# rossumur/espflix

Hardware: AMD Instinct MI355X
Metric: MPEG-1 352x192 frames/s (higher is better)
Workload: dtype u8/int32; 1 GPU; 1024 streams/GPU x GOP(12) I+11P, 352x192 MPEG-1 ES resident in HBM, ids rank*1024.. per rank (BASELINE configs[2]; at 8 GPUs = configs[4], stream k on rank floor(k*8/8192)); streams_per_gpu=1024, streams_total=1024, es_bytes_per_gpu=46457181, parallelism=stream-partition x1, coefficients_per_gpu=44531885, ring_depth=2

## Files before the change

### espflix_amd/csrc/efx_api.hip

```cpp
#include <hip/hip_runtime.h>

#include <algorithm>
#include <memory>
#include <mutex>
#include <thread>

#include <cstdio>
#include <cstdlib>
#include <cstring>
#include <string>
#include <vector>

#include "efx.h"
#include "efx_internal.h"
#include "enc_core.h"
#include "parse_tm.h"
#include "sbc_enc_core.h"

namespace efx {
struct DemuxChunk;
__global__ void k_demux_scan(const uint8_t*, const uint64_t*, const uint32_t*, const uint32_t*, DemuxChunk*);
__global__ void k_demux_offsets(const uint32_t*, const uint32_t*, DemuxChunk*, uint8_t*, const uint64_t*, uint32_t*, uint32_t*);
__global__ void k_demux(const uint8_t*, const uint64_t*, const uint32_t*, const uint32_t*, const DemuxChunk*, uint8_t*, PesEntry*);
__global__ void k_demux_fused(const uint8_t*, const uint64_t*, const uint32_t*, const uint32_t*, DemuxChunk*, uint8_t*, PesEntry*, uint32_t*, uint32_t*,
                              uint32_t*);
__global__ void k_demux_audio_scan(const uint8_t*, const uint64_t*, const uint32_t*, const uint32_t*, DemuxChunk*);
__global__ void k_demux_audio_offsets(const uint32_t*, const uint32_t*, DemuxChunk*, uint32_t*);
__global__ void k_demux_audio(const uint8_t*, const uint64_t*, const uint32_t*, const uint32_t*, const DemuxChunk*, uint8_t*, const uint64_t*);
__global__ void k_ts_sequences(const uint8_t*, const uint64_t*, const uint32_t*, const uint32_t*, PesEntry*, IdxInfo*);
__global__ void k_idx_bins(const PesEntry*, const uint32_t*, const IdxInfo*, uint32_t, uint32_t*, size_t);
__global__ void k_index(const uint8_t*, const uint64_t*, int, PicInfo*, SliceTmp*, uint32_t*, uint32_t*, uint32_t*,
                        const uint32_t*, const PesEntry*, const uint32_t*, const uint32_t*, int64_t*, int64_t*, int, int, int);
__global__ void k_advance(StreamState*, const uint32_t*, int64_t*, const int64_t*, int, int, int, int32_t*);
__global__ void k_slice_scan(const PicInfo*, const uint32_t*, int, int, const uint32_t*, uint32_t*, DecodeCounters*);
__global__ void k_slice_emit(const PicInfo*, const SliceTmp*, const uint32_t*, const uint64_t*, const uint32_t*, int, int,
                             const uint32_t*, SliceDesc*, uint32_t*);
__global__ void k_parse(const uint8_t*, const SliceDesc*, DecodeCounters*, const TmTables*, MbRec*, TmU4*, uint32_t*, uint32_t*,
                        int, int);
__global__ void k_recon(const MbRec*, const uint32_t*, const uint32_t*, const uint32_t*, uint8_t*, int, int, int, const int32_t*, int, int);
__global__ void k_recon_all(const MbRec*, const uint32_t*, const uint32_t*, const uint32_t*, uint8_t*, int, int, int, const int32_t*, int, int,
                            int, uint32_t*, uint32_t*, int);

__global__ void k_frame_hash(const uint8_t*, int, uint64_t*);
__global__ void k_fill(uint32_t*, uint32_t, size_t);
__global__ void k_composite(const uint8_t*, const VideoTables*, const VideoLineTemplates*, FieldArgs, uint16_t*);
__global__ void k_pdm(const int16_t*, int, int, int32_t*, uint16_t*);
template <int FMT, int CHROMA>
__global__ void k_export(const uint8_t*, int, ExportArgs);
__global__ void k_enc_begin(EncArgs);
__global__ void k_enc_rows(EncArgs);
__global__ void k_enc_pack(EncArgs);
__global__ void k_sbc(const uint8_t*, size_t, int, int, SbcState*, const SbcTables*, int16_t*, size_t, uint32_t*, uint32_t*, int);
__global__ void k_sbc_frames(const uint8_t*, size_t, int, int, SbcFrameInfo*, uint32_t*, uint32_t*, SbcQueues*);
__global__ void k_sbc_plan(const SbcFrameInfo*, int, int, const SbcState*, SbcFramePlan*, uint32_t*, SbcQueues*, uint32_t*, int, int, uint32_t*,
                           uint32_t*, SbcExtraItem*, uint8_t*);
__global__ void k_sbc_par_stereo(const uint8_t*, size_t, int, int, const SbcState*, SbcState*, const SbcTables*, const SbcFrameInfo*, int16_t*,
                                 size_t, uint32_t*, int, SbcQueues*, const uint32_t*, int, const SbcExtraItem*, int);
__global__ void k_sbc_par_mono(const uint8_t*, size_t, int, int, const SbcState*, SbcState*, const SbcTables*, const SbcFrameInfo*, int16_t*,
                               size_t, uint32_t*, int, SbcQueues*, const uint32_t*, int, const SbcExtraItem*, int);
__global__ void k_sbc_gen(const uint8_t*, size_t, int, int, const SbcState*, SbcState*, const SbcTables*, const SbcFrameInfo*,
                          const SbcFramePlan*, int16_t*, size_t, int, SbcQueues*, const uint32_t*, int, const uint8_t*, int);
__global__ void k_sbc_finish(const uint8_t*, size_t, int, int, SbcState*, const SbcState*, const SbcTables*, int16_t*, size_t, uint32_t*,
                             uint32_t*, int, uint32_t*);
__global__ void k_sbc_enc(SbcEncArgs);
__global__ void k_sbc_enc_state(SbcEncArgs);
__global__ void k_mux(MuxArgs);
}

using namespace efx;

#ifndef EFX_SBC_WG_PER_CU
#define EFX_SBC_WG_PER_CU 4
#endif

#ifndef EFX_PARSE_STREAMS
#define EFX_PARSE_STREAMS 2
#endif
#ifndef EFX_SLOTS
#define EFX_SLOTS 3
#endif
constexpr int kParseStreams = EFX_PARSE_STREAMS;
constexpr int kMaxGroups = 16;
static_assert(kMaxGroups <= kExportMaxGroups, "k_export takes every reconstruction group of a call");
#ifndef EFX_RECON_MERGE
#define EFX_RECON_MERGE 1
#endif
constexpr int kReconMerge = EFX_RECON_MERGE;
#ifndef EFX_GROUP_STREAMS
#define EFX_GROUP_STREAMS 1024
#endif
constexpr int kGroupStreams = EFX_GROUP_STREAMS;
constexpr int kTimingRing = 64;
constexpr int kSlots = EFX_SLOTS;
constexpr int kUploads = 3;
constexpr size_t kReconSyncWords(size_t streams) { return (64 + streams) * 32; }

struct efx_ctx {
    efx_config cfg{};
    hipStream_t stream = nullptr;
    bool own_stream = false;
    bool pooled_streams = false;
    unsigned stream_serial = 0;
    std::string err;

    size_t es_cap = 0;
    bool decoded = false, results_valid = false;

    ParseTables* d_tables = nullptr;
    TmTables* d_tm_tables = nullptr;
    uint8_t* d_frames = nullptr;
    StreamState* d_state = nullptr;

    struct Upload {
        uint8_t* d_es = nullptr;
        uint64_t* d_stream_off = nullptr;
        uint32_t* d_stream_perm = nullptr;
        uint32_t* d_ts_len = nullptr;
        uint32_t* d_pkt_base = nullptr;
        uint32_t* d_es_len = nullptr;
        uint32_t* d_pes_count = nullptr;
        PesEntry* d_pes = nullptr;
        uint8_t* h_es = nullptr;
        uint8_t* h_meta = nullptr;
        std::vector<uint64_t> stream_off;
        std::vector<uint32_t> es_len;
        int n_streams = 0;
        int sort_groups = 1;
        size_t es_used = 0, ts_bytes = 0;
        bool ts_input = false, valid = false;
        hipEvent_t uploaded = nullptr;
        hipEvent_t last_read[kParseStreams] = {};
        hipEvent_t ev_demux[2] = {nullptr, nullptr};
        bool demux_timed = false;
    } up[kUploads];
    int cur_up = -1;
    struct Arena {
        uint8_t* base;
        size_t bytes;
        bool owned;
    };
    std::vector<Arena> arenas;
    hipStream_t copy_stream = nullptr;
    uint8_t* d_ts = nullptr;
    DemuxChunk* d_demux_chunks = nullptr;
    size_t pes_cap = 0;
    IdxInfo* d_idx_info = nullptr;
    uint64_t* d_ts_off = nullptr;
    uint32_t* d_idx_len = nullptr;
    uint32_t* d_idx_base = nullptr;
    PesEntry* d_idx_seq = nullptr;
    bool ts_ready = false;

    struct Slot {
        uint32_t* d_pic_count = nullptr;
        uint32_t* d_status = nullptr;
        DecodeCounters* d_counters = nullptr;
        MbRec* d_mbrecs = nullptr;
        TmU4* d_raw = nullptr;
        uint32_t* d_coefs = nullptr;
        PicInfo* d_pics = nullptr;
        SliceTmp* d_slices_tmp = nullptr;
        uint32_t* d_qtab = nullptr;
        uint32_t* d_slice_base = nullptr;
        SliceDesc* d_descs = nullptr;
        int64_t* d_pts = nullptr;
        int32_t* d_call_pos = nullptr;
        uint32_t* d_recon_sync = nullptr;
        hipEvent_t parse_done[kReconMerge] = {}, recon_done = nullptr, wrap_cleared = nullptr;
        int epoch = 0;
        int upload = 0;
    } slot[kSlots];
    struct TimingEvents {
        hipEvent_t ev[5] = {nullptr, nullptr, nullptr, nullptr, nullptr};
    };
    std::vector<TimingEvents> timing_ring;
    uint64_t timed_calls = 0;
    struct Group {
        int slot, first, count;
        int half0, halves;
    };
    Group groups[kMaxGroups];
    int n_groups = 0;
    hipEvent_t last_recon_done = nullptr;
    uint64_t recon_groups_unsynced = 0;
    int last_upload = 0;
    int last_n_streams = 0;
    bool last_ts_input = false;
    uint64_t subcalls = 0;
    uint64_t parse_calls = 0;
    uint8_t timing_groups[kTimingRing] = {};
    uint16_t timing_launches[kTimingRing] = {};
    uint16_t timing_leaders[kTimingRing] = {};
    hipStream_t parse_streams[kParseStreams] = {};
    VideoTables* d_video[2] = {nullptr, nullptr};
    VideoLineTemplates* d_video_lines[2] = {nullptr, nullptr};
    SbcTables* d_sbc_tables = nullptr;
    sbcenc::Tables* d_sbc_enc_tables = nullptr;
    uint32_t* d_mux_before = nullptr;
    size_t mux_before_cap = 0;
    int parse_wg_cap = 0;
    int opt_groups = 0;
    int opt_parse_cap = 0;
    int opt_recon_mode = 0;
    int opt_recon_waves = 0;
    int opt_recon_items = 16;
    int n_cus = 256;
    uint32_t* d_sbc_flags = nullptr;
    SbcState* d_sbc_next = nullptr;
    size_t sbc_flags_cap = 0;
    SbcFrameInfo* d_sbc_info = nullptr;
    SbcFramePlan* d_sbc_plan = nullptr;
    SbcExtraItem* d_sbc_extra = nullptr;
    uint8_t* d_sbc_cover = nullptr;
    size_t sbc_info_cap = 0;
    size_t sbc_gran_cap = 0;
    int opt_sbc_serial = 0;
    int opt_demux_fused = 0;
    bool sbc_flags_clean = false;
    uint64_t* d_hash = nullptr;

    EncState* d_enc_state = nullptr;
    uint8_t* d_enc_pics = nullptr;
    uint8_t* d_enc_slices = nullptr;
    uint32_t* d_enc_slice_len = nullptr;
    enc::Tables* d_enc_tables = nullptr;
    std::unique_ptr<enc::Tables> h_enc_tables;
    uint32_t* h_enc_full = nullptr;
    uint32_t* d_enc_full = nullptr;
    bool enc_ready = false;
    bool enc_started = false;
    uint32_t enc_generation = 0;
    int enc_n_streams = 0, enc_format = 0, enc_gop = 0;

    int n_streams = 0;
    std::vector<int64_t> h_pts;
    std::vector<uint32_t> h_pic_count, h_status;
    std::vector<int32_t> h_call_pos;
    DecodeCounters h_counters{};

    bool timing = false;
};

namespace {

struct StreamSet {
    hipStream_t recon = nullptr, parse[kParseStreams] = {}, copy = nullptr;
    unsigned serial = 0;
// ... 200 lines not shown
    if (ctx->cfg.max_stream_bytes == 0)
        ctx->cfg.max_stream_bytes = (size_t)16384 * cfg->max_pictures * cfg->max_streams;
    auto bail = [&](int code) {
        efx_destroy(ctx);
        return code;
    };
    if (hipSetDevice(cfg->device) != hipSuccess)
        return bail(EFX_ERR_NO_DEVICE);
    StreamSet pooled;
    if (!cfg->hip_stream && take_stream_set(cfg->device, &pooled)) {
        ctx->stream = pooled.recon;
        ctx->own_stream = true;
        for (int i = 0; i < kParseStreams; i++)
            ctx->parse_streams[i] = pooled.parse[i];
        ctx->copy_stream = pooled.copy;
        ctx->pooled_streams = true;
        ctx->stream_serial = pooled.serial;
    } else if (cfg->hip_stream)
        ctx->stream = (hipStream_t)cfg->hip_stream;
    else {
        if (hipStreamCreateWithFlags(&ctx->stream, hipStreamNonBlocking) != hipSuccess)
            return bail(EFX_ERR_DEVICE);
        ctx->own_stream = true;
        ctx->pooled_streams = true;
        std::lock_guard<std::mutex> lk(g_pool_guard);
        ctx->stream_serial = ++g_set_serial;
    }
    if (!ctx->parse_streams[0]) {
        int lo = 0, hi = 0;
        if (hipDeviceGetStreamPriorityRange(&lo, &hi) != hipSuccess)
            return bail(EFX_ERR_DEVICE);
        for (auto& ps : ctx->parse_streams)
            if (hipStreamCreateWithPriority(&ps, hipStreamNonBlocking, hi) != hipSuccess)
                return bail(EFX_ERR_DEVICE);
        if (hipStreamCreateWithFlags(&ctx->copy_stream, hipStreamNonBlocking) != hipSuccess)
            return bail(EFX_ERR_DEVICE);
        std::vector<hipStream_t> order = {ctx->stream};
        for (auto ps : ctx->parse_streams)
            order.push_back(ps);
        order.push_back(ctx->copy_stream);
        for (hipStream_t st : order) {
            hipLaunchKernelGGL(k_fill, dim3(1), dim3(64), 0, st, (uint32_t*)nullptr, 0u, (size_t)0);
            if (hipStreamSynchronize(st) != hipSuccess)
                return bail(EFX_ERR_DEVICE);
        }
    }
    const size_t n = (size_t)cfg->max_streams, P = (size_t)cfg->max_pictures, D = (size_t)ctx->cfg.ring_depth;
    ctx->es_cap = ctx->cfg.max_stream_bytes + n * (kEsTailBytes + 32) + kEsGuardBytes;
    ctx->es_cap = (ctx->es_cap + 255) & ~(size_t)255;
    if (ctx->es_cap * kCoefsPerEsByte >= 0xFFFFFFFFull)
        return bail(EFX_ERR_CAPACITY);
    hipError_t e = hipSuccess;
    auto A = [&](hipError_t r) {
        if (e == hipSuccess)
            e = r;
    };
    A(dalloc(&ctx->d_tables, 1));
    A(dalloc(&ctx->d_tm_tables, 1));
    A(dalloc(&ctx->d_state, n));
    for (auto& u : ctx->up) {
        A(dalloc(&u.d_es, ctx->es_cap));
        A(dalloc(&u.d_stream_off, n + 1));
        A(dalloc(&u.d_stream_perm, n));
        A(hipHostMalloc(reinterpret_cast<void**>(&u.h_es), ctx->es_cap, hipHostMallocDefault));
        A(hipHostMalloc(reinterpret_cast<void**>(&u.h_meta), meta_bytes(n), hipHostMallocDefault));
        A(hipEventCreateWithFlags(&u.uploaded, hipEventDisableTiming));
        for (auto& ev : u.last_read)
            A(hipEventCreateWithFlags(&ev, hipEventDisableTiming));
        if (e == hipSuccess)
            A(hipMemset(u.d_es, 0, ctx->es_cap));
    }
    for (auto& sl : ctx->slot) {
        A(dalloc(&sl.d_pic_count, n));
        A(dalloc(&sl.d_status, n));
        A(dalloc(&sl.d_counters, kMaxGroups));
        A(dalloc(&sl.d_mbrecs, n * P * kMbCount));
        A(dalloc(&sl.d_raw, n * P * kMbCount));
        A(dalloc(&sl.d_coefs, ctx->es_cap * kCoefsPerEsByte));
        A(dalloc(&sl.d_pics, n * P));
        A(dalloc(&sl.d_slices_tmp, n * P * kMaxSlicesPerPicture));
        A(dalloc(&sl.d_qtab, n * P * 64));
        A(dalloc(&sl.d_slice_base, n * P + kMaxGroups));
        A(dalloc(&sl.d_descs, n * P * kMaxSlicesPerPicture));
        A(dalloc(&sl.d_call_pos, 2 * n));
        A(dalloc(&sl.d_recon_sync, kReconSyncWords(n)));
    }
    A(dalloc(&ctx->d_frames, n * D * kFrameBytes + 8192));
    A(dalloc(&ctx->d_video[0], 1));
    A(dalloc(&ctx->d_video[1], 1));
    A(dalloc(&ctx->d_video_lines[0], 1));
    A(dalloc(&ctx->d_video_lines[1], 1));
    A(dalloc(&ctx->d_hash, n * D));
    A(dalloc(&ctx->d_sbc_tables, 1));
    A(dalloc(&ctx->d_sbc_enc_tables, 1));
    if (e != hipSuccess) {
        fprintf(stderr, "efx_create: %s\n", hipGetErrorString(e));
        return bail(EFX_ERR_DEVICE);
    }
    {
        hipDeviceProp_t prop;
        if (hipGetDeviceProperties(&prop, cfg->device) == hipSuccess) {
            ctx->parse_wg_cap = std::max(1, prop.multiProcessorCount * 5 / 8);
            ctx->n_cus = std::max(1, prop.multiProcessorCount);
        }
        if (const char* v = getenv("EFX_GROUPS"))
            ctx->opt_groups = atoi(v);
        if (const char* v = getenv("EFX_FORCE_PARSE_CAP"))
            ctx->opt_parse_cap = atoi(v);
        if (const char* v = getenv("EFX_RECON_MODE"))
            ctx->opt_recon_mode = atoi(v);
        if (const char* v = getenv("EFX_RECON_WAVES"))
            ctx->opt_recon_waves = atoi(v);
        if (const char* v = getenv("EFX_DEMUX_FUSED"))
            ctx->opt_demux_fused = atoi(v) != 0;
        if (const char* v = getenv("EFX_RECON_ITEMS"))
            ctx->opt_recon_items = atoi(v);
        if (const char* cap = getenv("EFX_PARSE_WG_CAP"))
            ctx->parse_wg_cap = atoi(cap);
    }
    ParseTables* pt = new ParseTables;
    build_parse_tables(pt);
    A(hipMemcpy(ctx->d_tables, pt, sizeof(ParseTables), hipMemcpyHostToDevice));
    {
        TmTables* tt = new TmTables;
        build_tm_tables(tt);
        hipError_t e_tm = hipMemcpy(ctx->d_tm_tables, tt, sizeof(TmTables), hipMemcpyHostToDevice);
        delete tt;
        A(e_tm);
    }
    delete pt;
    for (int ntsc = 0; ntsc < 2; ntsc++) {
        VideoTables vt;
        build_video_tables(ntsc, &vt);
        A(hipMemcpy(ctx->d_video[ntsc], &vt, sizeof(vt), hipMemcpyHostToDevice));
        VideoLineTemplates* lt = new VideoLineTemplates;
        build_video_line_templates(&vt, lt);
        A(hipMemcpy(ctx->d_video_lines[ntsc], lt, sizeof(*lt), hipMemcpyHostToDevice));
        delete lt;
    }
    {
        SbcTables st;
        build_sbc_tables(&st);
        A(hipMemcpy(ctx->d_sbc_tables, &st, sizeof(st), hipMemcpyHostToDevice));
        sbcenc::Tables et;
        sbcenc::build_tables(&et);
        A(hipMemcpy(ctx->d_sbc_enc_tables, &et, sizeof(et), hipMemcpyHostToDevice));
    }
    A(hipMemset(ctx->d_frames, 0, n * D * kFrameBytes));
    for (auto& sl : ctx->slot) {
        A(hipMemset(sl.d_mbrecs, 0, n * P * kMbCount * sizeof(MbRec)));
        for (auto& ev : sl.parse_done)
            A(hipEventCreateWithFlags(&ev, hipEventDisableTiming));
        A(hipEventCreateWithFlags(&sl.recon_done, hipEventDisableTiming));
        A(hipEventCreateWithFlags(&sl.wrap_cleared, hipEventDisableTiming));
    }
    if (e != hipSuccess)
        return bail(EFX_ERR_DEVICE);
    *out = ctx;
    if (efx_reset(ctx) != EFX_OK || hipStreamSynchronize(ctx->stream) != hipSuccess) {
        *out = nullptr;
        return bail(EFX_ERR_DEVICE);
    }
    return EFX_OK;
}

void efx_destroy(efx_ctx* ctx)
{
    bind_device(ctx);
    if (!ctx)
        return;
    if (ctx->copy_stream)
        (void)hipStreamSynchronize(ctx->copy_stream);
    for (auto ps : ctx->parse_streams)
        if (ps)
            (void)hipStreamSynchronize(ps);
    if (ctx->stream)
        (void)hipStreamSynchronize(ctx->stream);
    for (auto& a : ctx->arenas) {
        if (a.owned)
            (void)hipHostFree(a.base);
        else
            (void)hipHostUnregister(a.base);
    }
    void* bufs[] = {ctx->d_tables, ctx->d_tm_tables, ctx->d_sbc_flags, ctx->d_sbc_next, ctx->d_sbc_info, ctx->d_sbc_plan, ctx->d_sbc_extra, ctx->d_sbc_cover, ctx->d_state, ctx->d_frames, ctx->d_video[0],  ctx->d_video[1], ctx->d_video_lines[0],
                    ctx->d_video_lines[1], ctx->d_hash, ctx->d_ts, ctx->d_demux_chunks, ctx->d_sbc_tables, ctx->d_idx_info, ctx->d_ts_off, ctx->d_idx_len,
                    ctx->d_idx_base, ctx->d_idx_seq, ctx->d_enc_state, ctx->d_enc_pics, ctx->d_enc_slices, ctx->d_enc_slice_len,
                    ctx->d_enc_tables, ctx->d_sbc_enc_tables, ctx->d_mux_before};
    if (ctx->h_enc_full)
        (void)hipHostFree(ctx->h_enc_full);
    for (auto& te : ctx->timing_ring)
        for (auto& ev : te.ev)
            if (ev)
                (void)hipEventDestroy(ev);
    for (void* b : bufs)
        if (b)
            (void)dev_free(b);
    for (auto& u : ctx->up) {
        void* ub[] = {u.d_es, u.d_stream_off, u.d_stream_perm, u.d_ts_len, u.d_pkt_base, u.d_es_len, u.d_pes_count, u.d_pes};
        for (void* b : ub)
            if (b)
                (void)dev_free(b);
        if (u.h_es)
            (void)hipHostFree(u.h_es);
        if (u.h_meta)
            (void)hipHostFree(u.h_meta);
        hipEvent_t evs[] = {u.uploaded, u.ev_demux[0], u.ev_demux[1]};
        for (auto ev : evs)
            if (ev)
                (void)hipEventDestroy(ev);
        for (auto ev : u.last_read)
            if (ev)
                (void)hipEventDestroy(ev);
    }
    for (auto& sl : ctx->slot) {
        void* sb[] = {sl.d_pic_count, sl.d_status, sl.d_counters, sl.d_mbrecs, sl.d_raw, sl.d_coefs, sl.d_pts, sl.d_call_pos, sl.d_recon_sync,
                      sl.d_pics,      sl.d_slices_tmp, sl.d_qtab, sl.d_slice_base, sl.d_descs};
        for (void* b : sb)
            if (b)
                (void)dev_free(b);
        for (auto ev : sl.parse_done)
            if (ev)
                (void)hipEventDestroy(ev);
        if (sl.recon_done)
            (void)hipEventDestroy(sl.recon_done);
        if (sl.wrap_cleared)
            (void)hipEventDestroy(sl.wrap_cleared);
    }
    bool complete = ctx->own_stream && ctx->stream && ctx->copy_stream;
    for (auto ps : ctx->parse_streams)
        complete = complete && ps;
    if (ctx->pooled_streams && complete) {
        StreamSet set;
        set.recon = ctx->stream;
        for (int i = 0; i < kParseStreams; i++)
            set.parse[i] = ctx->parse_streams[i];
        set.copy = ctx->copy_stream;
        set.serial = ctx->stream_serial;
        park_stream_set(ctx->cfg.device, set);
    } else {
        for (auto ps : ctx->parse_streams)
            if (ps)
                (void)hipStreamDestroy(ps);
        if (ctx->copy_stream)
            (void)hipStreamDestroy(ctx->copy_stream);
        if (ctx->own_stream && ctx->stream)
            (void)hipStreamDestroy(ctx->stream);
    }
    delete ctx;
}


static int ensure_ts_buffers(efx_ctx* ctx)
{
    if (ctx->ts_ready)
        return EFX_OK;
    if (ctx->d_ts)
        return fail(ctx, EFX_ERR_DEVICE, "transport-stream buffers: an earlier allocation failed");
    const size_t n_max = (size_t)ctx->cfg.max_streams;
    ctx->pes_cap = ctx->es_cap / 188 + n_max;
    hipError_t e = dalloc(&ctx->d_ts, ctx->es_cap);
    if (e == hipSuccess)
        e = dev_alloc(reinterpret_cast<void**>(&ctx->d_demux_chunks), (ctx->pes_cap / kDemuxChunk + n_max + 2) * 16 + n_max * sizeof(uint32_t));
    for (auto& u : ctx->up) {
        if (e == hipSuccess) e = dalloc(&u.d_ts_len, n_max);
        if (e == hipSuccess) e = dalloc(&u.d_pkt_base, n_max);
        if (e == hipSuccess) e = dalloc(&u.d_es_len, n_max);
        if (e == hipSuccess) e = dalloc(&u.d_pes_count, n_max);
        if (e == hipSuccess) e = dalloc(&u.d_pes, ctx->pes_cap);
        for (auto& ev : u.ev_demux)
            if (e == hipSuccess) e = hipEventCreate(&ev);
    }
    if (e == hipSuccess) e = dalloc(&ctx->d_idx_info, n_max);
    if (e == hipSuccess) e = dalloc(&ctx->d_ts_off, n_max + 1);
    if (e == hipSuccess) e = dalloc(&ctx->d_idx_len, n_max);
    if (e == hipSuccess) e = dalloc(&ctx->d_idx_base, n_max);
    if (e == hipSuccess) e = dalloc(&ctx->d_idx_seq, ctx->pes_cap);
    for (auto& sl : ctx->slot)
        if (e == hipSuccess) e = dalloc(&sl.d_pts, n_max * (size_t)ctx->cfg.max_pictures + n_max);
    if (e != hipSuccess)
        return fail(ctx, EFX_ERR_DEVICE, "transport-stream buffers", e);
    ctx->ts_ready = true;
    return EFX_OK;
}

static int upload_streams(efx_ctx* ctx, int n_streams, const uint8_t* const* data, const size_t* len, int format, bool in_place)
{
    bind_device(ctx);
    if (!ctx || !data || !len || n_streams <= 0 || (format != EFX_FORMAT_ES && format != EFX_FORMAT_TS))
        return fail(ctx, EFX_ERR_ARG, "efx_upload_streams: bad argument");
    if (n_streams > ctx->cfg.max_streams)
        return fail(ctx, EFX_ERR_CAPACITY, "efx_upload_streams: more streams than max_streams");
    const bool is_ts = format == EFX_FORMAT_TS;
    if (is_ts) {
        int r = ensure_ts_buffers(ctx);
        if (r)
            return r;
    }
    static const uint8_t tail[kEsTailBytes] = {0, 0, 0, 1, 0xB7, 0, 0, 1, 0xB7};
    std::vector<uint64_t> stream_off((size_t)n_streams + 1, 0);
// ... 396 lines not shown
    if (newest_pts)
        *newest_pts = st.pts_carry;
    return EFX_OK;
}

int efx_erase_frames(efx_ctx* ctx)
{
    bind_device(ctx);
    if (!ctx)
        return EFX_ERR_ARG;
    size_t bytes = (size_t)ctx->cfg.max_streams * ctx->cfg.ring_depth * kFrameBytes;
    EFX_HIP(hipMemsetAsync(ctx->d_frames, 0x30, bytes, ctx->stream));
    return EFX_OK;
}

int efx_decode_from(efx_ctx* ctx, int first_picture) { return efx_decode_range(ctx, first_picture, ctx ? ctx->cfg.max_pictures : 0); }

int efx_decode_range(efx_ctx* ctx, int first_picture, int n_pictures)
{
    bind_device(ctx);
    if (!ctx || first_picture < 0 || n_pictures < 1 || n_pictures > ctx->cfg.max_pictures)
        return EFX_ERR_ARG;
    if (ctx->cur_up < 0)
        return fail(ctx, EFX_ERR_STATE, "efx_decode: no streams uploaded");
    efx_ctx::Upload& u = ctx->up[ctx->cur_up];
    const int n_all = u.n_streams, P = ctx->cfg.max_pictures, D = ctx->cfg.ring_depth;
    const bool idle_at_call = ctx->recon_groups_unsynced == 0;
    const int G = ctx->opt_groups > 0 ? std::min(std::min(ctx->opt_groups, kMaxGroups), std::max(1, n_all / 8))
                                      : (idle_at_call ? group_count(n_all) : 1);
    {
        bool nested = true;
        for (int g = 1; g < G && nested; g++) {
            bool found = false;
            for (int k = 0; k <= u.sort_groups && !found; k++)
                found = group_first(n_all, u.sort_groups, k) == group_first(n_all, G, g);
            nested = found;
        }
        if (!nested) {
            int r = sync_all(ctx);
            if (r)
                return r;
            std::vector<uint32_t> perm((size_t)n_all);
            for (int i = 0; i < n_all; i++)
                perm[i] = (uint32_t)i;
            auto len_of = [&](uint32_t i) { return u.stream_off[i + 1] - u.stream_off[i]; };
            for (int g = 0; g < G; g++)
                std::stable_sort(perm.begin() + group_first(n_all, G, g), perm.begin() + group_first(n_all, G, g + 1),
                                 [&](uint32_t a, uint32_t b) { return len_of(a) > len_of(b); });
            EFX_HIP(hipMemcpy(u.d_stream_perm, perm.data(), perm.size() * sizeof(uint32_t), hipMemcpyHostToDevice));
            u.sort_groups = G;
        }
    }
    hipStream_t sr = ctx->stream;
    int timing_slot = -1;
    if (ctx->timing && !ctx->timing_ring.empty()) {
        timing_slot = (int)(ctx->timed_calls++ % kTimingRing);
        ctx->timing_groups[timing_slot] = (uint8_t)G;
        ctx->timing_leaders[timing_slot] = 0;
        ctx->timing_launches[timing_slot] = (uint16_t)(((G + kReconMerge - 1) / kReconMerge) * (ctx->opt_recon_mode == 0 ? n_pictures : 1));
    }
    ctx->last_upload = ctx->cur_up;
    ctx->last_n_streams = u.n_streams;
    ctx->last_ts_input = u.ts_input;
    const int R = (G + kReconMerge - 1) / kReconMerge;
    ctx->n_groups = R;
    for (int r = 0; r < R; r++) {
        const int h0 = r * kReconMerge, h1 = std::min(G, h0 + kReconMerge);
        const int rs0 = group_first(n_all, G, h0), rn = group_first(n_all, G, h1) - rs0;
        const int slot = (int)(ctx->subcalls++ % kSlots);
        ctx->groups[r] = {slot, rs0, rn, h0, h1 - h0};
        efx_ctx::Slot& sl = ctx->slot[slot];
        sl.upload = ctx->cur_up;
        const bool wrap = ++sl.epoch > 255;
        if (wrap)
            sl.epoch = 1;
        efx_ctx::TimingEvents* te0 = nullptr;
        for (int g = h0; g < h1; g++) {
            const int s0 = group_first(n_all, G, g), n = group_first(n_all, G, g + 1) - s0;
            const int pi = (int)(ctx->parse_calls++ % kParseStreams);
            hipStream_t sp = ctx->parse_streams[pi];
            DecodeCounters* counters = sl.d_counters + g;
            uint32_t* slice_base = sl.d_slice_base + (size_t)s0 * P + g;
            SliceDesc* descs = sl.d_descs + (size_t)s0 * P * kMaxSlicesPerPicture;

            EFX_HIP(hipStreamWaitEvent(sp, u.uploaded, 0));
            EFX_HIP(hipStreamWaitEvent(sp, sl.recon_done, 0));
            if (wrap && g == h0) {
                EFX_HIP(hipMemsetAsync(sl.d_mbrecs, 0, (size_t)ctx->cfg.max_streams * P * kMbCount * sizeof(MbRec), sp));
                EFX_HIP(hipEventRecord(sl.wrap_cleared, sp));
            } else if (wrap)
                EFX_HIP(hipStreamWaitEvent(sp, sl.wrap_cleared, 0));
            efx_ctx::TimingEvents* te = timing_slot >= 0 ? &ctx->timing_ring[(size_t)timing_slot * kMaxGroups + g] : nullptr;
            if (te && !te->ev[0])
                for (auto& ev : te->ev)
                    EFX_HIP(hipEventCreate(&ev));
            if (g == h0)
                te0 = te;
            if (te)
                EFX_HIP(hipEventRecord(te->ev[0], sp));
            hipLaunchKernelGGL(k_index, dim3(n), dim3(64 * kIndexWaves), 0, sp, u.d_es, u.d_stream_off, P, sl.d_pics, sl.d_slices_tmp,
                               sl.d_pic_count, sl.d_status, sl.d_qtab, ctx->d_tables->scan, u.d_pes, u.d_pkt_base, u.d_pes_count,
                               u.ts_input ? sl.d_pts : nullptr, u.ts_input ? sl.d_pts + (size_t)ctx->cfg.max_streams * P : nullptr,
                               first_picture, s0, n_pictures);
            hipLaunchKernelGGL(k_slice_scan, dim3(1), dim3(1024), 0, sp, sl.d_pics, sl.d_pic_count, n, P, u.d_stream_perm + s0,
                               slice_base, counters);
            hipLaunchKernelGGL(k_slice_emit, dim3((n * P * kMaxSlicesPerPicture + 255) / 256), dim3(256), 0, sp, sl.d_pics,
                               sl.d_slices_tmp, sl.d_pic_count, u.d_stream_off, slice_base, n, P, u.d_stream_perm + s0, descs, sl.d_status);
            if (te)
                EFX_HIP(hipEventRecord(te->ev[1], sp));
            const int max_slices = n * P * kMaxSlicesPerPicture;
            const int parse_waves = (max_slices + kParseLanes - 1) / kParseLanes;
            int parse_wgs = (parse_waves + kParseWaves - 1) / kParseWaves;
            const bool recon_busy = ctx->opt_parse_cap == 1 || (ctx->opt_parse_cap == 0 && ctx->recon_groups_unsynced > 0);
            if (ctx->parse_wg_cap > 0 && recon_busy)
                parse_wgs = std::min(parse_wgs, ctx->parse_wg_cap);
            hipLaunchKernelGGL(k_parse, dim3(parse_wgs), dim3(64 * kParseWaves), 0, sp, u.d_es,
                               descs, counters, ctx->d_tm_tables, sl.d_mbrecs, sl.d_raw, sl.d_coefs, sl.d_status, P, sl.epoch);
            if (te)
                EFX_HIP(hipEventRecord(te->ev[2], sp));
            EFX_HIP(hipEventRecord(sl.parse_done[g - h0], sp));
            EFX_HIP(hipEventRecord(u.last_read[pi], sp));
        }

        for (int g = h0; g < h1; g++)
            EFX_HIP(hipStreamWaitEvent(sr, sl.parse_done[g - h0], 0));
        if (te0) {
            EFX_HIP(hipEventRecord(te0->ev[4], sr));
            ctx->timing_leaders[timing_slot] |= (uint16_t)(1u << h0);
        }
        hipLaunchKernelGGL(k_advance, dim3((rn + 255) / 256), dim3(256), 0, sr, ctx->d_state, sl.d_pic_count,
                           u.ts_input ? sl.d_pts : nullptr, u.ts_input ? sl.d_pts + (size_t)ctx->cfg.max_streams * P : nullptr, rs0, rn,
                           P, sl.d_call_pos);
        constexpr int kGroupsPerPicture = (kMbCount * 6 + 63) / 64;
#ifdef EFX_RECON_ITEMS2
        constexpr int kReconGridY = (kGroupsPerPicture + 1) / 2;
#else
        constexpr int kReconGridY = kGroupsPerPicture;
#endif
        if (ctx->opt_recon_mode == 0) {
            for (int p = 0; p < n_pictures; p++)
                hipLaunchKernelGGL(k_recon, dim3(rn, kReconGridY), dim3(64), 0, sr, sl.d_mbrecs, sl.d_coefs,
                                   ctx->d_tables->scan, sl.d_qtab, ctx->d_frames, P, D, p, sl.d_call_pos, sl.epoch, rs0);
        } else if (rn > 0) {
            EFX_HIP(hipMemsetAsync(sl.d_recon_sync, 0, kReconSyncWords((size_t)rn) * sizeof(uint32_t), sr));
            const long long items = (long long)rn * kGroupsPerPicture * n_pictures;
            const int per_cu = ctx->opt_recon_waves > 0 ? ctx->opt_recon_waves : 18;
            const long long waves = ctx->opt_recon_items > 0 ? (items + ctx->opt_recon_items - 1) / ctx->opt_recon_items
                                                             : std::min<long long>(items, (long long)ctx->n_cus * per_cu);
            hipLaunchKernelGGL(k_recon_all, dim3((unsigned)waves), dim3(64), 0, sr, sl.d_mbrecs,
                               sl.d_coefs, ctx->d_tables->scan, sl.d_qtab, ctx->d_frames, P, D, n_pictures, sl.d_call_pos, sl.epoch, rs0, rn,
                               sl.d_recon_sync, sl.d_status, ctx->opt_recon_items);
        }
        if (te0)
            EFX_HIP(hipEventRecord(te0->ev[3], sr));
        EFX_HIP(hipEventRecord(sl.recon_done, sr));
        ctx->last_recon_done = sl.recon_done;
        ctx->recon_groups_unsynced++;
    }
    EFX_HIP(hipGetLastError());
    ctx->decoded = true;
    ctx->results_valid = false;
    return EFX_OK;
}

int efx_decode(efx_ctx* ctx) { return efx_decode_from(ctx, 0); }

int efx_sync(efx_ctx* ctx)
{
    bind_device(ctx);
    if (!ctx)
        return EFX_ERR_ARG;
    return sync_all(ctx);
}

static int fetch_results(efx_ctx* ctx)
{
    if (!ctx->decoded)
        return fail(ctx, EFX_ERR_STATE, "no decode has run");
    if (ctx->results_valid)
        return EFX_OK;
    int r = sync_all(ctx);
    if (r)
        return r;
    const bool ts_input = ctx->last_ts_input;
    ctx->n_streams = ctx->last_n_streams;
    const size_t P = (size_t)ctx->cfg.max_pictures;
    ctx->h_pic_count.resize(ctx->n_streams);
    ctx->h_status.resize(ctx->n_streams);
    ctx->h_call_pos.resize(2 * (size_t)ctx->n_streams);
    if (ts_input)
// ... 1015 lines not shown
```

### espflix_amd/csrc/efx_internal.h

```cpp
#pragma once
#include <cstdint>

namespace efx {

constexpr int kMbW = 22, kMbH = 12, kMbCount = 264;
constexpr int kStride = 528, kStripBytes = 8448, kFrameBytes = 101376;
constexpr int kMaxSlicesPerPicture = 16;
#ifndef EFX_PARSE_LANES
#define EFX_PARSE_LANES 64
#endif
constexpr int kParseLanes = EFX_PARSE_LANES;
#ifndef EFX_PARSE_WAVES
#define EFX_PARSE_WAVES 4
#endif
constexpr int kParseWaves = EFX_PARSE_WAVES;
constexpr int kIndexWaves = 4;
constexpr int kMaxUnitsPerStream = 4096;
constexpr int kCoefsPerEsByte = 4;
constexpr int kEsTailBytes = 9;
constexpr int kEsGuardBytes = 512;

struct PicInfo {
    uint32_t first_slice;
    uint16_t n_slices;
    uint8_t type;
    uint8_t full_pel;
    uint8_t r_size;
    uint8_t custom_q;
    uint16_t reserved;
    uint32_t seq_off;
    uint32_t start_off;
};

struct PesEntry {
    uint32_t es_off;
    uint32_t reserved;
    int64_t pts;
};

struct StreamState {
    uint32_t fb_index;
    uint32_t pts_seen;
    int64_t pts_carry;
};

constexpr int64_t kNoPts = INT64_MIN;

struct SliceTmp {
    uint32_t off;
    uint32_t len_code;
};

struct SliceDesc {
    uint32_t es_off;
    uint32_t es_len;
    uint32_t stream;
    uint32_t pic_code_flags;
    uint32_t mb_limit;
    uint32_t reserved;
};

struct MbRec {
    uint32_t coef_base;
    uint8_t cnt[6];
    uint8_t flags;
    uint8_t epoch;
    int16_t mvx, mvy;
};
static_assert(sizeof(MbRec) == 16, "MbRec must be 16 bytes");


struct ParseTables {
    uint32_t scan[64];
};

struct DecodeCounters {
    uint32_t total_slices;
    uint32_t streams;
    unsigned long long coefficients;
    unsigned long long macroblocks;
    uint32_t next_wave;
    uint32_t reserved;
};

struct VideoTables {
    int32_t line_width, line_count, hsync, hsync_long, hsync_short, burst_start, burst_width, active_start;
    int32_t pal;
    uint16_t sync_level, blanking_level, black_level, pad;
    int16_t burst0[64], burst1[64];
    uint32_t color_tab[768];
};

constexpr int kCompositeItemsPerBlock = 2048;
constexpr int kLineTemplates = 6;
constexpr int kLineTemplateWidth = 1152;
struct VideoLineTemplates {
    uint16_t tpl[kLineTemplates][kLineTemplateWidth];
};
void build_video_line_templates(const VideoTables* v, VideoLineTemplates* out);

constexpr int kExportItemsPerPicture = 22 * 96;
constexpr int kExportItemsPerBlock = 1024;
constexpr int kExportMaxGroups = 16;

struct ExportArgs {
    int first_stream, ring_depth;
    int slot;
    int picture;
    int n_groups;
    int group_first[kExportMaxGroups];
    const int32_t* call_pos[kExportMaxGroups];
    int full_range;
    uint8_t* dst;
    size_t dst_stride;
};

struct IdxInfo {
    int64_t first_pts, last_pts;
    uint32_t n_seq;
    uint32_t fast;
};

struct FieldArgs {
    int first_stream, ring_depth;
    int slot, other_slot;
    int frame_counter;
    int hscroll;
    const uint8_t* overlay;
    size_t overlay_stride;
    int overlay_scale;
    int overlay_progress;
};

#ifndef EFX_DEMUX_CHUNK
#define EFX_DEMUX_CHUNK 16
#endif
constexpr int kDemuxChunk = EFX_DEMUX_CHUNK;
#ifndef EFX_DEMUX_THREADS
#define EFX_DEMUX_THREADS 64
#endif
constexpr int kDemuxThreads = EFX_DEMUX_THREADS;
constexpr uint32_t kDemuxFailedFlag = 0x80000000u;
static_assert(kDemuxChunk % 4 == 0 && kDemuxChunk >= 4 && kDemuxChunk <= 256, "k_demux stages whole 16-byte groups");
// ... 115 lines not shown
```

### espflix_amd/csrc/k_index.hip

```cpp
#include <hip/hip_runtime.h>

#include "efx_internal.h"
#include "efx.h"

namespace efx {

namespace {

__device__ inline uint32_t wave_excl_scan(uint32_t v, uint32_t* total)
{
    uint32_t x = v;
    int lane = threadIdx.x & 63;
#pragma unroll
    for (int d = 1; d < 64; d <<= 1) {
        uint32_t y = __shfl_up(x, d, 64);
        if (lane >= d)
            x += y;
    }
    *total = __shfl(x, 63, 64);
    return x - v;
}

__device__ inline uint32_t load_bits(const uint8_t* p, uint32_t bitpos, int n)
{
// ... 393 lines not shown
            }
        }
        uint32_t mine = 0;
#pragma unroll
        for (int r = 0; r < kRun; r++)
            mine += v[r];
        uint32_t tot;
        uint32_t ex = wave_excl_scan(mine, &tot);
        if (lane == 63)
            wave_tot[wv] = tot;
        __syncthreads();
        uint32_t off = carry;
        for (int k = 0; k < wv; k++)
            off += wave_tot[k];
        uint32_t at = off + ex;
#pragma unroll
        for (int r = 0; r < kRun; r++) {
            const int i = base + tid * kRun + r;
            if (i < n)
                slice_base[i] = at;
            at += v[r];
        }
        __syncthreads();
        if (tid == 1023)
            carry = at;
        __syncthreads();
    }
    if (tid == 0) {
        counters->total_slices = carry;
        counters->streams = (uint32_t)n_streams;
        counters->coefficients = 0;
        counters->macroblocks = 0;
        counters->next_wave = 0;
        slice_base[n] = carry;
    }
}

__global__ __launch_bounds__(256) void k_slice_emit(const PicInfo* __restrict__ pics,
                                                    const SliceTmp* __restrict__ slices_tmp,
                                                    const uint32_t* __restrict__ pic_count,
                                                    const uint64_t* __restrict__ stream_off,
                                                    const uint32_t* __restrict__ slice_base, int n_streams,
                                                    int max_pictures, const uint32_t* __restrict__ stream_perm,
                                                    SliceDesc* __restrict__ descs, uint32_t* __restrict__ status)
{
    int t = blockIdx.x * blockDim.x + threadIdx.x;
    int k = t % kMaxSlicesPerPicture, i = t / kMaxSlicesPerPicture;
    if (i >= n_streams * max_pictures)
        return;
    int p = i / n_streams, s = (int)stream_perm[i - p * n_streams];
    if ((uint32_t)p >= pic_count[s])
        return;
    PicInfo pi = pics[(size_t)s * max_pictures + p];
    if (k >= pi.n_slices)
        return;
    SliceTmp st = slices_tmp[(size_t)s * max_pictures * kMaxSlicesPerPicture + pi.first_slice + k];
    SliceDesc d;
    d.es_off = (uint32_t)stream_off[s] + st.off;
    d.es_len = st.len_code >> 8;
    d.stream = (uint32_t)s;
    d.pic_code_flags = (uint32_t)p | ((st.len_code & 0xFF) << 8) | ((uint32_t)pi.type << 16) | ((uint32_t)pi.full_pel << 18) |
                       ((uint32_t)pi.r_size << 19) | ((uint32_t)pi.custom_q << 22);
    uint32_t limit = kMbCount;
    bool out_of_order = false;
    {
        const uint32_t code = st.len_code & 0xFF;
        const SliceTmp* all = slices_tmp + (size_t)s * max_pictures * kMaxSlicesPerPicture + pi.first_slice;
        for (int j = 0; j < (int)pi.n_slices; j++) {
            const uint32_t other = all[j].len_code & 0xFF;
            if (other > code && (other - 1) * kMbW < limit)
                limit = (other - 1) * kMbW;
            if (other == code && j > k)
                limit = 0;
            out_of_order |= j < k && other >= code;
        }
    }
    if (out_of_order)
        atomicOr(&status[s], EFX_STREAM_SLICE_ORDER);
    d.mb_limit = limit;
    d.reserved = 0;
    descs[slice_base[i] + k] = d;
}

}
```

Measured before the change: 9.053 million frames/s.

## Sort slice descriptors by descending size before parse to balance work

Adds a k_slice_sort kernel that reorders each picture-index segment of slice descriptors with a stable counting sort keyed on ES length, largest first. Slices whose mb_limit makes them empty get key zero and go to the end. The intent is that long slices are scheduled first in k_parse, cutting tail imbalance across workgroups. In exchange it adds one kernel launch, an extra descriptor buffer and an extra read and write pass over the descriptors.

```diff
diff --git a/espflix_amd/csrc/efx_api.hip b/espflix_amd/csrc/efx_api.hip
--- a/espflix_amd/csrc/efx_api.hip
+++ b/espflix_amd/csrc/efx_api.hip
@@ -35,6 +35,7 @@
 __global__ void k_slice_scan(const PicInfo*, const uint32_t*, int, int, const uint32_t*, uint32_t*, DecodeCounters*);
 __global__ void k_slice_emit(const PicInfo*, const SliceTmp*, const uint32_t*, const uint64_t*, const uint32_t*, int, int,
                              const uint32_t*, SliceDesc*, uint32_t*);
+__global__ void k_slice_sort(const SliceDesc*, const uint32_t*, int, SliceDesc*);
 __global__ void k_parse(const uint8_t*, const SliceDesc*, DecodeCounters*, const TmTables*, MbRec*, TmU4*, uint32_t*, uint32_t*,
                         int, int);
 __global__ void k_recon(const MbRec*, const uint32_t*, const uint32_t*, const uint32_t*, uint8_t*, int, int, int, const int32_t*, int, int);
@@ -163,6 +164,7 @@
         uint32_t* d_qtab = nullptr;
         uint32_t* d_slice_base = nullptr;
         SliceDesc* d_descs = nullptr;
+        SliceDesc* d_descs_emit = nullptr;
         int64_t* d_pts = nullptr;
         int32_t* d_call_pos = nullptr;
         uint32_t* d_recon_sync = nullptr;
@@ -529,6 +531,7 @@
         A(dalloc(&sl.d_qtab, n * P * 64));
         A(dalloc(&sl.d_slice_base, n * P + kMaxGroups));
         A(dalloc(&sl.d_descs, n * P * kMaxSlicesPerPicture));
+        A(dalloc(&sl.d_descs_emit, n * P * kMaxSlicesPerPicture));
         A(dalloc(&sl.d_call_pos, 2 * n));
         A(dalloc(&sl.d_recon_sync, kReconSyncWords(n)));
     }
@@ -661,7 +664,7 @@
     }
     for (auto& sl : ctx->slot) {
         void* sb[] = {sl.d_pic_count, sl.d_status, sl.d_counters, sl.d_mbrecs, sl.d_raw, sl.d_coefs, sl.d_pts, sl.d_call_pos, sl.d_recon_sync,
-                      sl.d_pics,      sl.d_slices_tmp, sl.d_qtab, sl.d_slice_base, sl.d_descs};
+                      sl.d_pics,      sl.d_slices_tmp, sl.d_qtab, sl.d_slice_base, sl.d_descs, sl.d_descs_emit};
         for (void* b : sb)
             if (b)
                 (void)dev_free(b);
@@ -1224,6 +1227,7 @@
             DecodeCounters* counters = sl.d_counters + g;
             uint32_t* slice_base = sl.d_slice_base + (size_t)s0 * P + g;
             SliceDesc* descs = sl.d_descs + (size_t)s0 * P * kMaxSlicesPerPicture;
+            SliceDesc* descs_emit = sl.d_descs_emit + (size_t)s0 * P * kMaxSlicesPerPicture;
 
             EFX_HIP(hipStreamWaitEvent(sp, u.uploaded, 0));
             EFX_HIP(hipStreamWaitEvent(sp, sl.recon_done, 0));
@@ -1247,7 +1251,8 @@
             hipLaunchKernelGGL(k_slice_scan, dim3(1), dim3(1024), 0, sp, sl.d_pics, sl.d_pic_count, n, P, u.d_stream_perm + s0,
                                slice_base, counters);
             hipLaunchKernelGGL(k_slice_emit, dim3((n * P * kMaxSlicesPerPicture + 255) / 256), dim3(256), 0, sp, sl.d_pics,
-                               sl.d_slices_tmp, sl.d_pic_count, u.d_stream_off, slice_base, n, P, u.d_stream_perm + s0, descs, sl.d_status);
+                               sl.d_slices_tmp, sl.d_pic_count, u.d_stream_off, slice_base, n, P, u.d_stream_perm + s0, descs_emit, sl.d_status);
+            hipLaunchKernelGGL(k_slice_sort, dim3(P), dim3(64 * kSliceSortWaves), 0, sp, descs_emit, slice_base, n, descs);
             if (te)
                 EFX_HIP(hipEventRecord(te->ev[1], sp));
             const int max_slices = n * P * kMaxSlicesPerPicture;
diff --git a/espflix_amd/csrc/efx_internal.h b/espflix_amd/csrc/efx_internal.h
--- a/espflix_amd/csrc/efx_internal.h
+++ b/espflix_amd/csrc/efx_internal.h
@@ -15,6 +15,7 @@
 #endif
 constexpr int kParseWaves = EFX_PARSE_WAVES;
 constexpr int kIndexWaves = 4;
+constexpr int kSliceSortWaves = 8;
 constexpr int kMaxUnitsPerStream = 4096;
 constexpr int kCoefsPerEsByte = 4;
 constexpr int kEsTailBytes = 9;
@@ -59,6 +60,19 @@
     uint32_t mb_limit;
     uint32_t reserved;
 };
+
+constexpr uint32_t kSliceKeyShift = 4, kSliceKeyBins = 1024;
+#if defined(__HIPCC__)
+__host__ __device__
+#endif
+inline uint32_t slice_order_key(uint32_t es_len, uint32_t pic_code_flags, uint32_t mb_limit)
+{
+    const uint32_t first_mb = (((pic_code_flags >> 8) & 0xFF) - 1) * (uint32_t)kMbW;
+    if ((int)mb_limit <= (int)first_mb)
+        return 0;
+    const uint32_t k = es_len >> kSliceKeyShift;
+    return k < kSliceKeyBins - 1 ? k : kSliceKeyBins - 1;
+}
 
 struct MbRec {
     uint32_t coef_base;
diff --git a/espflix_amd/csrc/k_index.hip b/espflix_amd/csrc/k_index.hip
--- a/espflix_amd/csrc/k_index.hip
+++ b/espflix_amd/csrc/k_index.hip
@@ -499,4 +499,83 @@
     descs[slice_base[i] + k] = d;
 }
 
-}
+static_assert(kSliceKeyBins == 2 * 64 * kSliceSortWaves, "k_slice_sort's prefix pass: a thread owns two bins");
+static_assert(kSliceKeyBins == 1 << 10, "k_slice_sort matches keys with ten ballots");
+
+__global__ __launch_bounds__(64 * kSliceSortWaves) void k_slice_sort(const SliceDesc* __restrict__ src,
+                                                                const uint32_t* __restrict__ slice_base, int n_streams,
+                                                                SliceDesc* __restrict__ dst)
+{
+    __shared__ uint32_t bins[kSliceSortWaves][kSliceKeyBins];
+    __shared__ uint32_t wave_tot[kSliceSortWaves];
+    const int tid = threadIdx.x, lane = tid & 63, wave = tid >> 6;
+    const uint32_t seg0 = slice_base[(size_t)blockIdx.x * n_streams], seg1 = slice_base[(size_t)(blockIdx.x + 1) * n_streams];
+    if (seg1 <= seg0)
+        return;
+    const uint32_t len = seg1 - seg0;
+    const uint32_t run = (len + 64 * kSliceSortWaves - 1) / (64 * kSliceSortWaves) * 64;
+    const uint32_t r0 = min((uint32_t)wave * run, len), r1 = min(r0 + run, len);
+    const SliceDesc* seg = src + seg0;
+    auto key_of = [](const SliceDesc& d) { return slice_order_key(d.es_len, d.pic_code_flags, d.mb_limit); };
+
+    for (int i = tid; i < kSliceSortWaves * (int)kSliceKeyBins; i += 64 * kSliceSortWaves)
+        (&bins[0][0])[i] = 0;
+    __syncthreads();
+    for (uint32_t i = r0 + lane; i < r1; i += 64)
+        atomicAdd(&bins[wave][key_of(seg[i])], 1u);
+    __syncthreads();
+    {
+        uint32_t v[2][kSliceSortWaves], mine = 0;
+#pragma unroll
+        for (int j = 0; j < 2; j++)
+#pragma unroll
+            for (int w = 0; w < kSliceSortWaves; w++) {
+                v[j][w] = bins[w][kSliceKeyBins - 1 - (2 * tid + j)];
+                mine += v[j][w];
+            }
+        uint32_t tot;
+        const uint32_t ex = wave_excl_scan(mine, &tot);
+        if (lane == 0)
+            wave_tot[wave] = tot;
+        __syncthreads();
+        uint32_t at = ex;
+        for (int w = 0; w < wave; w++)
+            at += wave_tot[w];
+#pragma unroll
+        for (int j = 0; j < 2; j++)
+#pragma unroll
+            for (int w = 0; w < kSliceSortWaves; w++) {
+                bins[w][kSliceKeyBins - 1 - (2 * tid + j)] = at;
+                at += v[j][w];
+            }
+    }
+    __syncthreads();
+    const uint64_t lt = (1ull << lane) - 1;
+    SliceDesc next = {};
+    if (r0 + lane < r1)
+        next = seg[r0 + lane];
+    for (uint32_t i0 = r0; i0 < r1; i0 += 64) {
+        const SliceDesc d = next;
+        const bool valid = i0 + lane < r1;
+        if (i0 + 64 + lane < r1)
+            next = seg[i0 + 64 + lane];
+        const uint32_t key = valid ? key_of(d) : 0u;
+        uint64_t same = __ballot(valid);
+#pragma unroll
+        for (int b = 0; b < 10; b++) {
+            const bool bit = (key >> b) & 1;
+            const uint64_t m = __ballot(bit);
+            same &= bit ? m : ~m;
+        }
+        const int first = same ? __ffsll((unsigned long long)same) - 1 : 0;
+        uint32_t base = 0;
+        if (valid && lane == first)
+            base = atomicAdd(&bins[wave][key], (uint32_t)__popcll(same));
+        base = __shfl(base, first, 64);
+        const uint32_t pos = base + (uint32_t)__popcll(same & lt);
+        if (valid && pos < len)
+            dst[seg0 + pos] = d;
+    }
+}
+
+}
```

Result: faster. 9.311 million frames/s (median of 6 runs) (+2.8%).
